# Nashatyrev/shadow

Measured on AMD Instinct MI355X. Metric: APSP wall time + source-SSSPs/sec, 10k-vertex GML graph, 1/2/4/8 MI355X, higher is better.
Workload: dtype u32+f32

## Files before the change

include/shadow_routing.h:

```cpp
#ifndef SHADOW_ROUTING_H
#define SHADOW_ROUTING_H

#include <stddef.h>
#include <stdint.h>

#ifdef __cplusplus
extern "C" {
#endif

#define SRG_OK 0
#define SRG_ERR_ARG 1
#define SRG_ERR_NO_EDGE 2
#define SRG_ERR_MULTI_EDGE 3
#define SRG_ERR_UNREACHABLE 4
#define SRG_ERR_LATENCY_RANGE 5
#define SRG_ERR_HIP 6
#define SRG_ERR_OOM 7
#define SRG_ERR_PARSE 8
#define SRG_ERR_RCCL 9
#define SRG_ERR_INTERNAL 10

typedef struct srg_edge_list {
    uint32_t num_vertices;
    uint32_t directed;
// ... 74 lines not shown
#define SRG_OPT_H2D_CODEC 25
#define SRG_OPT_EDGE_SHARD 29
#define SRG_OPT_LATE_LOSS 30
#define SRG_OPT_FW_LINE_SPLIT 31
#define SRG_OPT_FW_STEP 32
#define SRG_OPT_FW_OVERLAP 33
#define SRG_OPT_TEST_FAULT 34
#define SRG_OPT_TABLE_POOL_BYTES 35
#define SRG_OPT_TABLE_POOL_IDLE_BYTES 36
#define SRG_OPT_CREATE_MS_RUNTIME 37
#define SRG_OPT_CREATE_MS_LIBRARY 38
#define SRG_OPT_FW_XCD_ORDER 39
#define SRG_OPT_SCAN_MIRROR 40
#define SRG_OPT_SCAN_MIRRORED 41
#define SRG_OPT_SCAN_MIRROR_CAP 42
int srg_set_option(srg_ctx* ctx, int option, double value);
int srg_get_option(srg_ctx* ctx, int option, double* value);

int srg_compute_shortest_paths(srg_ctx* ctx, const srg_edge_list* graph,
                               const uint32_t* nodes, uint32_t num_nodes,
                               uint64_t* out_latency_ns, float* out_packet_loss,
                               srg_stats* stats, char* errbuf, size_t errlen);

int srg_compute_shortest_paths_device(srg_ctx* ctx, const srg_edge_list* graph_dev,
                                      const uint32_t* nodes_dev, uint32_t num_nodes,
                                      uint64_t* out_latency_ns_dev, float* out_packet_loss_dev,
                                      void* hip_stream, srg_stats* stats,
                                      char* errbuf, size_t errlen);

int srg_get_direct_paths(srg_ctx* ctx, const srg_edge_list* graph,
// ... 124 lines not shown
```

shadow_amd/_native.py:

```python
import ctypes
import os

_HERE = os.path.dirname(os.path.abspath(__file__))
LIB_PATH = os.path.join(_HERE, "libshadow_routing.so")

SRG_OK = 0
SRG_ERR_ARG = 1
SRG_ERR_NO_EDGE = 2
SRG_ERR_MULTI_EDGE = 3
SRG_ERR_UNREACHABLE = 4
SRG_ERR_LATENCY_RANGE = 5
SRG_ERR_HIP = 6
SRG_ERR_OOM = 7
SRG_ERR_PARSE = 8
SRG_ERR_RCCL = 9
SRG_ERR_INTERNAL = 10
SRG_ERR_EVENT_ORDER = 11

SRG_PATH_DENSE_U32 = 0
SRG_PATH_DENSE_U64 = 1
SRG_PATH_DIRECT = 2
SRG_PATH_SPARSE_U32 = 3
SRG_PATH_SPARSE_U64 = 4

# ... 13 lines not shown
SRG_OPT_H2D_CODEC = 25
SRG_OPT_EDGE_SHARD = 29
SRG_OPT_LATE_LOSS = 30
SRG_OPT_FW_LINE_SPLIT = 31
SRG_OPT_FW_STEP = 32
SRG_OPT_FW_OVERLAP = 33
SRG_OPT_TEST_FAULT = 34
SRG_OPT_TABLE_POOL_BYTES = 35
SRG_OPT_TABLE_POOL_IDLE_BYTES = 36
SRG_OPT_CREATE_MS_RUNTIME = 37
SRG_OPT_CREATE_MS_LIBRARY = 38
SRG_OPT_FW_XCD_ORDER = 39
SRG_OPT_SCAN_MIRROR = 40
SRG_OPT_SCAN_MIRRORED = 41
SRG_OPT_SCAN_MIRROR_CAP = 42
SRG_ALGO_AUTO = 0
SRG_ALGO_DENSE = 1
SRG_ALGO_SPARSE = 2
SRG_UNIQUE_ID_BYTES = 128

SRG_SCAN_NONE = 0
SRG_SCAN_SPARSE = 1
SRG_SCAN_DENSE = 2

_u32p = ctypes.POINTER(ctypes.c_uint32)
_u64p = ctypes.POINTER(ctypes.c_uint64)
_f32p = ctypes.POINTER(ctypes.c_float)


class EdgeList(ctypes.Structure):
# ... 249 lines not shown
```

shadow_amd/csrc/dense.hip.h:

```cpp
template <class K, int T>
bool run_dense(srg_ctx& c, const DevGraph& g, const Plan& pl, const uint32_t* nodes, uint32_t n, uint64_t* out_lat,
               float* out_loss, hipStream_t st, const Prelude& P, srg_stats* stats, HostSink* sink,
               FwOverlap* ov = nullptr) {
    const bool pre = ov && ov->on && ov->ok && ov->ended && sizeof(K) == 4 && T == FwOverlap::T;
    if (sizeof(K) == 8 && c.kout_key) {
        if (!(sink && sink->widen)) fail(SRG_INTERNAL_NEED_U64, "the build needs u64 latency keys: no u32 key table");
        sink->widen = false;
        c.kout_key = nullptr;
        c.kout_diag = nullptr;
    }
    const uint32_t V = g.V;
    const size_t Vp = ((size_t)V + T - 1) / T * T;
    const size_t VV = Vp * Vp;
    const bool multi = c.comm && c.comm->nranks > 1;
    Timer tm(st);
    c.own_row0 = pl.p0;
    c.own_row1 = pl.p1;

    K* W = (K*)c.b_W.get(VV * sizeof(K));
    uint32_t* WL = (uint32_t*)c.b_WL.get(VV * 4);
    K* D = (K*)c.b_D.get(VV * sizeof(K));
    bool wl_late = false;
    if (pre) {
        wl_late = g.late && !g.late->applied;
// ... 287 lines not shown
        const size_t Eb = E_layout + 256;
        uint32_t* cscpos = (uint32_t*)c.b_cscfill.get((size_t)nbTT5 * nK5 * V5_TT * 4);
        K* ent_w = (K*)c.b_entw.get(Eb * sizeof(K));
        uint2* ent_ub = (uint2*)c.b_grpe.get(Eb * 8);
        uint32_t* cscent = (uint32_t*)c.b_cscent.get(std::max<uint64_t>(E_ess, 1) * 4);
        k_v5_cscpos<<<(NT + 255) / 256, 256, 0, st>>>(v5_cnt, cscoff, NT, nK5, cscpos);
        uint2* rec = (uint2*)c.b_entkey.get((Eb + V5_SLACK) * 8);
        {
            const size_t nwaves = (size_t)nw64 * nK5;
            k_v5_fill<K><<<(unsigned)((nwaves * 64 + 255) / 256), 256, 0, st>>>(ess, W, WL, Vp, V, nw64, nK5, v5_cnt,
                                                                                  v5_goff, cscpos, rec, ent_w,
                                                                                  ent_ub, cscent);
        }
        HIP_CHECK(hipGetLastError());
        const size_t lds_rows = loss_rows_lds(V);
        bool mirror = c.scan_mirror && !g.directed && pl.G == 1 && !multi && !simulated && nloc == n && P.ident &&
                      !v5lo && lds_rows <= 150 * 1024;
        const uint32_t scan_groups = c.scan_groups ? (uint32_t)c.scan_groups : mirror ? 4u : 3u;
        const bool interleave = sink_rows && lds_rows <= 150 * 1024 && scan_groups > 1;
        if (interleave) set_lds(k_loss_rows<K, true>, lds_rows);
        uint32_t* PREDK = lds_rows <= 150 * 1024 ? (uint32_t*)c.b_PRED2.get(nmax * Vp * 8) : nullptr;
        auto pack_pred = [&](uint32_t r0, uint32_t r1) {
            const uint32_t nsb = (r1 - r0 + 127) / 128, nt8 = (nbTT5 + 7) / 8;
            k_pred_pack<<<8u * nt8 * nsb, 256, 0, st>>>(PRED, Vp, r0, r1, NT, nbTT5, nsb, ent_ub, (uint2*)PREDK,
                                                        multi_cnt, mirror ? 1u : 0u);
            HIP_CHECK(hipGetLastError());
        };
        auto mirror_rows = [&](uint32_t r0, uint32_t r1) {
            if (r1 <= r0 || r1 <= SB) return;
            const size_t pairs = (size_t)(r1 - r0) * Vp, room = std::min<size_t>(pairs / 2, (size_t)1 << 30);
            const uint32_t cap = (uint32_t)std::min<size_t>(
                room, c.scan_mirror_cap ? (size_t)c.scan_mirror_cap : std::max<size_t>(pairs / 1024, 256));
            uint2* work = (uint2*)(PRED + (size_t)r0 * Vp);
            HIP_CHECK(hipMemsetAsync(mirror_cnt, 0, 4, st));
            const uint32_t nlow = (r1 - 1) / SB * SB;
            k_pred_mirror<<<dim3(nlow / 64, (r1 - r0 + 63) / 64), 256, 0, st>>>((uint2*)PREDK, Vp, r0, r1, V, work, cap,
                                                                               mirror_cnt, multi_cnt);
            k_mirror_slow<K><<<1024, 256, 0, st>>>(work, mirror_cnt, cap, DST, npad, ent_ub, ent_w, cscoff, cscent,
                                                   (uint2*)PREDK, Vp, multi_cnt);
            HIP_CHECK(hipGetLastError());
        };
        std::vector<uint32_t> tri_h;
        if (nloc) HIP_CHECK(hipStreamWaitEvent(st, c.ev_dst, 0));
        for (bool again = nloc != 0; again;) {
            again = false;
            if (interleave) HIP_CHECK(hipMemsetAsync(&P.flags->changed, 0, 4, st));
            const uint32_t inf_check = v5lo ? 0u : 1u;
            const uint32_t nbS5 = (uint32_t)(npad / SB);
            const uint32_t ng = interleave ? std::min<uint32_t>(scan_groups, nbS5) : 1u;
            auto cut = [&](uint32_t q) { return mirror ? scan_group_cut_tri(q, ng, nbS5) : scan_group_cut(q, ng, nbS5); };
            const uint32_t* tri_d = nullptr;
            std::vector<size_t> tri_off(ng + 1, 0);
            if (mirror) {
                tri_h.clear();
                for (uint32_t gi = 0; gi < ng; ++gi) {
                    tri_scan_blocks(cut(gi), cut(gi + 1), nbTT5, tri_h);
                    tri_off[gi + 1] = tri_h.size();
                }
                uint32_t* d = (uint32_t*)c.b_tri.get(std::max<size_t>(tri_h.size(), 1) * 4);
                if (!tri_h.empty()) HIP_CHECK(hipMemcpyAsync(d, tri_h.data(), tri_h.size() * 4, hipMemcpyHostToDevice, st));
                HIP_CHECK(hipMemsetAsync(mirror_cnt, 0, 8, st));
                tri_d = d;
            }
            for (uint32_t gi = 0; gi < ng; ++gi) {
                const uint32_t c0 = cut(gi), c1 = cut(gi + 1);
                if (c1 == c0) continue;
                const uint32_t nblk = mirror ? (uint32_t)(tri_off[gi + 1] - tri_off[gi])
                                             : (nbTT5 + 3) / 4 * ((c1 - c0 + 7) / 8);
                if (nblk)
                    tight_v5<<<8u * 32u * ((nblk + 7) / 8), V5_WAVES * 64, 0, st>>>(
                        DSTs, npad, dsts_bytes, lnodes, nloc, V, NT, nbTT5, c1, nK5, c0, v5_goff,
                        (const uint32_t*)c.b_entkey.get(0), PRED, Vp, inf_check, mirror ? tri_d + tri_off[gi] : nullptr);
                HIP_CHECK(hipGetLastError());
                if (interleave) {
                    const uint32_t r0 = c0 * SB, r1 = std::min<uint32_t>(c1 * SB, nloc);
                    if (r1 <= r0) continue;
                    pack_pred(r0, r1);
                    if (mirror) mirror_rows(r0, r1);
                    k_loss_rows<K, true><<<r1 - r0, 1024, lds_rows, st>>>(PREDK, Vp, V, lnodes, nloc, ent_ub, ent_w,
                                                                   DST, npad, cscoff, cscent, P.selfloss, nodes, n,
                                                                   lpos, out_loss, &P.flags->changed, r0,
                                                                   mirror ? mirror_cnt + 1 : nullptr);
                    HIP_CHECK(hipGetLastError());
                    sink->send_rows(st, out_loss, sink->loss, pl.p0 + r0, r1 - r0, 4);
                }
            }
            if (!PREDK) k_count_multi<<<nloc, kThreads, 0, st>>>(PRED, nloc, V, Vp, multi_cnt);
            HIP_CHECK(hipGetLastError());
            ms_scan += tm.lap();
            if (interleave) {
                sink->loss_sent = true;
                rb_async(c, MS_CHANGED, &P.flags->changed, st);
                if (mirror) rb_async(c, MS_MIRROR, mirror_cnt + 1, st);
                HIP_CHECK(hipStreamSynchronize(st));
                rounds = (int)rb_get<uint32_t>(c, MS_CHANGED);
                loss_written = true;
            } else if (lds_rows <= 150 * 1024) {
                set_lds(k_loss_rows<K, true>, lds_rows);
                HIP_CHECK(hipMemsetAsync(&P.flags->changed, 0, 4, st));
                pack_pred(0, nloc);
                if (mirror) mirror_rows(0, nloc);
                const uint32_t nchunk = std::max<uint32_t>(1, std::min<uint32_t>(c.loss_chunks ? c.loss_chunks : sink_rows ? 8 : 1, nloc));
                for (uint32_t q = 0; q < nchunk; ++q) {
                    const uint32_t r0 = (uint32_t)((uint64_t)nloc * q / nchunk);
                    const uint32_t r1 = (uint32_t)((uint64_t)nloc * (q + 1) / nchunk);
                    if (r1 == r0) continue;
                    k_loss_rows<K, true><<<r1 - r0, 1024, lds_rows, st>>>(PREDK, Vp, V, lnodes, nloc, ent_ub, ent_w,
                                                                   DST, npad, cscoff, cscent, P.selfloss, nodes, n,
                                                                   lpos, out_loss, &P.flags->changed, r0,
                                                                   mirror ? mirror_cnt + 1 : nullptr);
                    HIP_CHECK(hipGetLastError());
                    if (sink_rows) sink->send_rows(st, out_loss, sink->loss, pl.p0 + r0, r1 - r0, 4);
                }
                if (sink_rows) sink->loss_sent = true;
                rb_async(c, MS_CHANGED, &P.flags->changed, st);
                if (mirror) rb_async(c, MS_MIRROR, mirror_cnt + 1, st);
                HIP_CHECK(hipStreamSynchronize(st));
                rounds = (int)rb_get<uint32_t>(c, MS_CHANGED);
                loss_written = true;
            } else {
                float* L0 = (float*)c.b_L0.get(nmax * Vp * 4);
                float* L1 = (float*)c.b_L1.get(nmax * Vp * 4);
// ... 103 lines not shown
```

shadow_amd/csrc/env_switches.h:

```cpp
#pragma once
#include <algorithm>
#include <cstddef>
#include <cstdlib>
#include <cstring>

namespace srg_env {

static inline bool is_set(const char* name) { return std::getenv(name) != nullptr; }
static inline bool first_char_is(const char* name, char ch) {
    const char* e = std::getenv(name);
    return e && e[0] == ch;
}
static inline bool equals(const char* name, const char* value) {
    const char* e = std::getenv(name);
    return e && std::strcmp(e, value) == 0;
}

static inline bool stream_hops_events() { return equals("SRG_STREAM_HOPS", "events"); }
static inline int fw_bulk_q() {
    const char* e = std::getenv("SRG_FW_BULK_Q");
    return !e ? -1 : e[0] == '0' ? 0 : e[0] == '1' ? 1 : -1;
}
static inline bool debug_overlap() { return is_set("SRG_DEBUG_OVERLAP"); }
static inline int debug_sparse() {
    const char* e = std::getenv("SRG_DEBUG_SPARSE");
    return !e ? 0 : e[0] == '2' ? 2 : 1;
}
static inline bool debug_codec() { return is_set("SRG_DEBUG_CODEC"); }
static inline bool debug_create() { return is_set("SRG_DEBUG_CREATE"); }
static inline bool sparse_kernel_bf() { return equals("SRG_SPARSE_KERNEL", "bf"); }
static inline bool sparse_split_off() { return first_char_is("SRG_SPARSE_SPLIT", '0'); }
static inline bool latency_unit_ns() { return equals("SRG_LATENCY_UNIT", "1"); }
static inline int codec_threads() {
// ... 15 lines not shown
```

shadow_amd/csrc/plan.h:

```cpp
#pragma once
#include <algorithm>
#include <cstddef>
#include <cstdint>
#include <vector>

namespace {

struct Plan {
    int G = 1, g = 0, nb = 0, rb0 = 0, rb1 = 0;
    std::vector<int> blk_lo;
    uint32_t p0 = 0, p1 = 0;
    std::vector<uint32_t> lnodes, lpos;
    int owner(int b) const { return (int)(std::upper_bound(blk_lo.begin(), blk_lo.end(), b) - blk_lo.begin()) - 1; }
    bool own(int b) const { return b >= rb0 && b < rb1; }
};

inline void tri_tile_h(int nb, int idx, int& I, int& J) {
    int i = 0;
    while (i + 1 < nb && (i + 1) * nb - (i + 1) * i / 2 <= idx) ++i;
    I = i;
    J = i + (idx - (i * nb - i * (i - 1) / 2));
}

inline Plan make_plan(int G, int g, uint32_t V, int T, const std::vector<uint32_t>& nodes_h) {
// ... 72 lines not shown
    if (q == 0) return 0u;
    if (q >= ng) return nblocks;
    const uint32_t last = nblocks ? (nblocks - 1) / 8 * 8 : 0u;
    const bool tail = ng >= 3 && last > 0;
    const uint32_t end = tail ? last : nblocks;
    const uint32_t parts = tail ? ng - 1 : ng;
    if (q >= parts) return end;
    const uint64_t want = tri_scan_work(end, nblocks) / 2;
    uint32_t c = 0;
    while (c < end && tri_scan_work(c, nblocks) < want) ++c;
    const uint32_t half = std::min(end, (c + 4) / 8 * 8);
    if (q == 1) return half;
    return std::min(end, half + ((end - half) * (q - 1) / (parts - 1) + 4) / 8 * 8);
}

}
```

shadow_amd/csrc/routing.hip:

```cpp
#include <hip/hip_runtime.h>
#include <hsa/hsa.h>
#include <hsa/hsa_ext_amd.h>
#include <sys/mman.h>

#include <algorithm>
#include <atomic>
#include <chrono>
#include <cmath>
#include <condition_variable>
#include <deque>
#include <cstdio>
#include <cstdlib>
#include <cstring>
#include <functional>
#include <map>
#include <memory>
#include <mutex>
#include <new>
#include <stdexcept>
#include <string>
#include <thread>
#include <vector>

#include "../../include/shadow_routing.h"
// ... 713 lines not shown
    Event ev_dst;
    int fw_line_split = 0;
    int fw_step = -1;
    DevBuf b_xlb, b_xflags;
    uint32_t xepoch = 0;
    std::vector<Event> ev_ov;
    uint32_t* kout_key = nullptr;
    uint64_t* kout_diag = nullptr;
    DevBuf b_odiag;
    int fw_overlap = 1;
    int fw_xcd_order = 1;
    int scan_mirror = 1;
    int scan_mirrored = 0;
    int scan_mirror_cap = 0;
    DevBuf b_tri;
    int test_fault = 0;
    std::shared_ptr<TablePool> tpool = std::make_shared<TablePool>();
    double ms_create_runtime = 0, ms_create_lib = 0;
    DevBuf b_ek0, b_ek1, b_eh0, b_eh1, b_ei0, b_ei1, b_ehist, b_eoffs, b_ered;
    ~srg_ctx() {
        delete comm;
        for (uint32_t* p : sig)
            if (p) (void)hipFree(p);
        if (h_lring) (void)hipHostFree(h_lring);
        if (hbox) (void)hipHostFree(hbox);
        for (hipStream_t s : {aux_stream, comm_stream, d2h_stream, stream})
            if (s) (void)hipStreamDestroy(s);
        delete pool;
        if (h_ring) (void)hipHostFree(h_ring);
        tpool->close();
// ... 77 lines not shown
                                      hipFuncAttributeMaxDynamicSharedMemorySize, (int)bytes));
}

constexpr int kMailSlots = 64;
template <class T>
void rb_async(srg_ctx& c, int slot, const T* dev, hipStream_t st) {
    static_assert(sizeof(T) <= 64, "mailbox slot");
    HIP_CHECK(hipMemcpyAsync(c.hbox + 64 * slot, dev, sizeof(T), hipMemcpyDeviceToHost, st));
}
template <class T>
T rb_get(const srg_ctx& c, int slot) {
    T v;
    std::memcpy(&v, c.hbox + 64 * slot, sizeof(T));
    return v;
}
enum MailSlot { MS_EDGESTATS, MS_FLAGS, MS_TIMEOUT, MS_REDUCE, MS_TAIL0, MS_TAIL1, MS_NMULTI, MS_CHANGED, MS_MIN, MS_REDUCE2, MS_MIRROR };

struct Prelude {
    EdgeStats es;
    uint32_t* selfcnt;
    uint64_t* selflat;
    float* selfloss;
    Flags* flags;
    std::vector<uint32_t> nodes_h;
    bool ident = false;
    bool range_risk = false;
    bool wrap_risk = false;
    uint64_t unit = 1;
    unsigned long long max_key = 0;
};

// ... 976 lines not shown
            fw->end(ms_xchg);
            ended = true;
        }
    }
};

#include "dense.hip.h"
#include "sparse_run.hip.h"

void compute_device(srg_ctx& c, const DevGraph& g, const uint32_t* nodes, uint32_t n, uint64_t* out_lat,
                    float* out_loss, hipStream_t st, srg_stats* stats, HostSink* sink = nullptr,
                    FwOverlap* ov = nullptr) {
    HIP_CHECK(hipStreamSynchronize(c.aux_stream));
    HIP_CHECK(hipStreamSynchronize(c.comm_stream));
    c.scan_mirrored = 0;
    if (g.V == 0) {
        if (n) fail(SRG_ERR_ARG, "nodes given for an empty graph");
        return;
    }
    const bool ov_fw = ov && ov->on && ov->ok && ov->begun;
    Prelude P = prelude(c, g, nodes, n, ov_fw ? c.comm_stream : st, true);
    if (n == 0) return;
    const uint64_t unit = (P.es.unit > 1 && !srg_env::latency_unit_ns()) ? P.es.unit : 1;
    P.unit = unit;
    const bool pre = ov && ov->on && ov->ok && ov->ended && P.es.max_lat < 0xFFFFFFFFull;
    if (pre) P.unit = 1;
    P.max_key = P.es.max_lat / P.unit;
    if (stats) stats->latency_unit_ns = P.unit;
    const unsigned __int128 bound = (unsigned __int128)P.max_key * (g.V > 1 ? g.V - 1 : 1);
    P.range_risk = bound >= ((unsigned __int128)1 << 62);
// ... 969 lines not shown
        lap("stream main");
        c->ms_create_runtime = ms_since(tcreate);
        const auto tlib = std::chrono::steady_clock::now();
        int prio_lo = 0, prio_hi = 0;
        HIP_CHECK(hipDeviceGetStreamPriorityRange(&prio_lo, &prio_hi));
        HIP_CHECK(hipStreamCreateWithPriority(&c->aux_stream, hipStreamNonBlocking, prio_hi));
        HIP_CHECK(hipStreamCreateWithFlags(&c->comm_stream, hipStreamNonBlocking));
        HIP_CHECK(hipStreamCreateWithFlags(&c->d2h_stream, hipStreamNonBlocking));
        lap("streams aux, comm, d2h");
        HIP_CHECK(hipHostMalloc((void**)&c->hbox, 64 * kMailSlots, hipHostMallocDefault));
        lap("mailbox");
        c->sdma.init(device);
        lap("sdma agents");
        c->loss_stream = c->d2h_stream;
        for (Event* e : {&c->ev_a, &c->ev_b, &c->ev_c, &c->ev_d, &c->ev_e, &c->ev_ledges, &c->ev_wlate, &c->ev_fwreset,
                         &c->ev_dst})
            e->create();
        int wv = 0;
        if (hipDeviceGetAttribute(&wv, hipDeviceAttributeCanUseStreamWaitValue, device) == hipSuccess && wv) {
            for (uint32_t*& p : c->sig) HIP_CHECK(hipExtMallocWithFlags((void**)&p, 8, hipMallocSignalMemory));
            HIP_CHECK(hipStreamWriteValue32(c->stream, c->sig[0], 0, 0));
            HIP_CHECK(hipStreamWriteValue32(c->stream, c->sig[1], 0, 0));
            HIP_CHECK(hipStreamSynchronize(c->stream));
        }
        lap("events, signals");
        if (!srg_env::create_warm_off()) {
            warm_context(*c);
            lap("warm-up (module, rings, copies)");
        }
        c->ms_create_lib = ms_since(tlib);
        std::lock_guard<std::mutex> lk(g_dev_mu);
// ... 93 lines not shown
#endif
            ctx->test_fault = (int)value;
            return SRG_OK;
        case SRG_OPT_FW_XCD_ORDER:
            if (value != 0 && value != 1) return SRG_ERR_ARG;
            ctx->fw_xcd_order = (int)value;
            return SRG_OK;
        case SRG_OPT_SCAN_MIRROR:
            if (value != 0 && value != 1) return SRG_ERR_ARG;
            ctx->scan_mirror = (int)value;
            return SRG_OK;
        case SRG_OPT_SCAN_MIRROR_CAP:
            if (!(value >= 0 && value <= 1073741824.0)) return SRG_ERR_ARG;
            ctx->scan_mirror_cap = (int)value;
            return SRG_OK;
        case SRG_OPT_TABLE_POOL_BYTES: {
            if (!(value >= 0.0 && value <= 1e15)) return SRG_ERR_ARG;
            std::lock_guard<std::mutex> pl(ctx->tpool->mu);
            ctx->tpool->limit = (size_t)value;
            ctx->tpool->max_idle = 0;
            ctx->tpool->trim_locked(ctx->tpool->limit);
            return SRG_OK;
        }
        case SRG_OPT_ALGORITHM:
            if (value != SRG_ALGO_AUTO && value != SRG_ALGO_DENSE && value != SRG_ALGO_SPARSE) return SRG_ERR_ARG;
            ctx->algorithm = (int)value;
            return SRG_OK;
        default:
            return SRG_ERR_ARG;
    }
// ... 26 lines not shown
            std::lock_guard<std::mutex> pl(ctx->tpool->mu);
            *value = (double)ctx->tpool->limit;
            break;
        }
        case SRG_OPT_TABLE_POOL_IDLE_BYTES: {
            std::lock_guard<std::mutex> pl(ctx->tpool->mu);
            *value = (double)ctx->tpool->idle_bytes;
            break;
        }
        case SRG_OPT_CREATE_MS_RUNTIME: *value = ctx->ms_create_runtime; break;
        case SRG_OPT_FW_XCD_ORDER: *value = ctx->fw_xcd_order; break;
        case SRG_OPT_CREATE_MS_LIBRARY: *value = ctx->ms_create_lib; break;
        case SRG_OPT_SCAN_MIRROR: *value = ctx->scan_mirror; break;
        case SRG_OPT_SCAN_MIRRORED: *value = ctx->scan_mirrored; break;
        case SRG_OPT_SCAN_MIRROR_CAP: *value = ctx->scan_mirror_cap; break;
        default: return SRG_ERR_ARG;
    }
    return SRG_OK;
}

void srg_destroy(srg_ctx* ctx) {
    if (!ctx) return;
    (void)hipSetDevice(ctx->device);
    {
        std::lock_guard<std::mutex> lk(g_dev_mu);
        --g_dev_ctx[ctx->device];
    }
    delete ctx;
}

// ... 424 lines not shown
```

shadow_amd/csrc/tight_sparse.hip.h:

```cpp
#pragma once
#include <hip/hip_runtime.h>
#include <stdint.h>

#include "kernels.hip.h"

namespace srg {

template <class K>
__global__ void __launch_bounds__(256) k_ess_mask(const K* __restrict__ W, const K* __restrict__ D, size_t ld,
                                                   uint32_t V, uint32_t u0, uint32_t u1, uint32_t nw64,
                                                   unsigned long long* __restrict__ ess) {
    const uint32_t lane = threadIdx.x & 63, wave = threadIdx.x >> 6;
    const uint32_t u = u0 + blockIdx.x;
    if (u >= u1) return;
    const K* Wu = W + (size_t)u * ld;
    const K* Du = D + (size_t)u * ld;
    unsigned long long* eu = ess + (size_t)u * nw64;
    if constexpr (sizeof(K) == 4) {
        for (uint32_t w0 = wave * 4; w0 < nw64; w0 += 16) {
            const uint32_t t = w0 * 64 + lane * 4;
            uint4 a = make_uint4(0u, 0u, 0u, 0u), d = make_uint4(1u, 1u, 1u, 1u);
            if (t < ld) {
                a = *reinterpret_cast<const uint4*>(Wu + t);
                d = *reinterpret_cast<const uint4*>(Du + t);
// ... 140 lines not shown
    if (j == V5_TW - 1) {
        const uint32_t total = incl;
        for (size_t q = 2 * ((size_t)pbase + total); q < 2 * (size_t)goff[g + 1]; ++q) {
            rec[q] = make_uint2(0u, KeyOps<uint32_t>::INF);
            ent_w[q] = KeyOps<K>::INF;
            ent_ub[q] = make_uint2(0u, __float_as_uint(1.0f));
        }
    }
}

typedef uint32_t v16u_v5 __attribute__((ext_vector_type(16)));
struct alignas(64) V5Grp {
    uint32_t v[16];
};

__global__ void __launch_bounds__(512, 4) tight_v5(const uint32_t* __restrict__ DST, size_t npad, uint32_t dst_bytes,
                                                    const uint32_t* __restrict__ nodes, uint32_t n, uint32_t V,
                                                    uint32_t NT, uint32_t nbTT, uint32_t nbS, uint32_t nK, uint32_t c0,
                                                    const uint32_t* __restrict__ goff, const uint32_t* __restrict__ rec,
                                                    uint32_t* __restrict__ PRED, size_t ldp, uint32_t inf_check,
                                                    const uint32_t* __restrict__ tri) {
    __shared__ __attribute__((aligned(16))) uint32_t rows[2 * V5_UC * V5_SB];
    const uint32_t bid = blockIdx.x, xcd = bid & 7, slot = bid >> 3;
    const uint32_t blk = (slot >> 5) * 8 + xcd, nbb = (nbTT + 3) / 4;
    uint32_t tb = blk % nbb, sg = blk / nbb;
    if (tri) {
        const uint32_t d = tri[blk];
        if (d == 0xFFFFFFFFu) return;
        tb = d & 0xFFFFu;
        sg = d >> 16;
    }
    const uint32_t b = tb * 4 + (slot & 3), c = c0 + sg * 8 + ((slot >> 2) & 7);
    if (c >= nbS || b >= nbTT) return;
    if (tri && b < c) return;
    const uint32_t tid = threadIdx.x, lane = tid & 63;
    const uint32_t wave = (uint32_t)__builtin_amdgcn_readfirstlane(tid >> 6);
    const uint32_t r0 = c * V5_SB + 2 * lane;
    const __amdgpu_buffer_rsrc_t rsrc = make_rsrc(DST, dst_bytes);
    const uint32_t t0 = b * V5_TT + wave * V5_TW;
// ... 88 lines not shown
    for (uint32_t h = 0; h < 2; ++h) {
        const uint32_t r = r0 + h;
        if (r >= n) continue;
        const uint32_t s = nodes[r];
        uint32_t o[V5_TW];
#pragma unroll
        for (uint32_t j = 0; j < V5_TW; ++j) {
            const uint32_t t = t0 + j;
            const uint32_t nd = h ? ndh[j] : ndl[j];
            const uint32_t st = h ? sth[j] : stl[j];
            o[j] = (t >= V || t == s || (inf_check && nd == 0u - KeyOps<uint32_t>::INF)) ? PRED_NONE : st;
        }
        uint4* out = reinterpret_cast<uint4*>(PRED + (size_t)r * ldp + t0);
#pragma unroll
        for (uint32_t j = 0; j < V5_TW; j += 4) out[j / 4] = make_uint4(o[j], o[j + 1], o[j + 2], o[j + 3]);
    }
}

__global__ void __launch_bounds__(256) k_pred_pack(const uint32_t* __restrict__ PRED, size_t ldp, uint32_t r0,
                                                   uint32_t r1, uint32_t NT, uint32_t nbTT, uint32_t nsb,
                                                   const uint2* __restrict__ ent_ub, uint2* __restrict__ PK,
                                                   unsigned long long* __restrict__ multi, uint32_t tri) {
    const uint32_t xcd = blockIdx.x & 7, slot = blockIdx.x >> 3;
    const uint32_t b = xcd + 8 * (slot / nsb), sb = slot % nsb;
    if (b >= nbTT) return;
    if (tri && b < r0 / V5_SB + sb) return;
    const uint32_t tx = threadIdx.x & 31, ty = threadIdx.x >> 5;
    const uint32_t t = b * V5_TT + tx * 4;
    const bool tv = t < NT;
    uint32_t nm = 0;
// ... 158 lines not shown
                const uint2 ub = ent_ub[e];
                if (KeyOps<K>::add(DST[(size_t)ub.x * npad + r], ent_w[e]) != dst) continue;
                const float cnd = fold_loss(Lrow[ub.x], __uint_as_float(ub.y));
                v = cnd < v ? cnd : v;
            }
        }
        Lout[r * ldp + t] = v;
        changed |= (v != Lrow[t]);
    }
    if (changed) atomicOr(changed_flag, 1u);
}

constexpr uint32_t U_SELF = 0xFFFFFFFFu, U_NONE = 0xFFFFFFFEu, U_MULTI = 0xFFFFFFFDu;
constexpr uint32_t U_MLIST = 0xF0000000u;
constexpr uint32_t LM_T = 32, LM_E = 16;
constexpr size_t loss_rows_lds(uint32_t V) { return (size_t)V * 12 + LM_T * (4 + 4 + LM_E * 8) + 16; }

template <class K, bool PK>
__global__ void __launch_bounds__(1024) k_loss_rows(const uint32_t* __restrict__ PRED, size_t ldp, uint32_t V,
                                                     const uint32_t* __restrict__ nodes, uint32_t n,
                                                     const uint2* __restrict__ ent_ub, const K* __restrict__ ent_w,
                                                     const K* __restrict__ DST, size_t npad,
                                                     const uint32_t* __restrict__ csc_off,
                                                     const uint32_t* __restrict__ csc_ent,
                                                     const float* __restrict__ self_loss,
                                                     const uint32_t* __restrict__ cols, uint32_t ncols,
                                                     const uint32_t* __restrict__ rowpos, float* __restrict__ out_loss,
                                                     uint32_t* __restrict__ max_sweeps, uint32_t row0,
                                                     const uint32_t* __restrict__ skip) {
    if (skip && *skip) return;
    extern __shared__ __attribute__((aligned(16))) unsigned char smem_raw[];
    uint32_t* U = reinterpret_cast<uint32_t*>(smem_raw);
    float* Bf = reinterpret_cast<float*>(U + V);
    float* L = Bf + V;
    uint32_t* m_t = reinterpret_cast<uint32_t*>(L + V);
    uint32_t* m_n = m_t + LM_T;
    uint32_t* m_u = m_n + LM_T;
    float* m_b = reinterpret_cast<float*>(m_u + LM_T * LM_E);
    __shared__ uint32_t changed, nm;
    const uint32_t r = row0 + blockIdx.x;
    const uint32_t s = nodes[r];
    const uint32_t* prow = PRED + (size_t)r * ldp * (PK ? 2 : 1);
    if (threadIdx.x == 0) nm = 0;
    if (threadIdx.x < LM_T) m_n[threadIdx.x] = 0;
    __syncthreads();
    for (uint32_t t = threadIdx.x; t < V; t += blockDim.x) {
        uint2 pk = make_uint2(0u, 0u);
        if constexpr (PK) pk = reinterpret_cast<const uint2*>(prow)[t];
        const uint32_t p = PK ? pk.x : prow[t];
        uint32_t u;
        float bb = 1.0f, l = 1.0f;
        if (t == s) {
            u = U_SELF;
            l = 0.0f;
        } else if (p == PRED_NONE) {
            u = U_NONE;
        } else if (p == PRED_MULTI) {
            const uint32_t i = atomicAdd(&nm, 1u);
            u = U_MULTI;
            if (i < LM_T) {
                m_t[i] = t;
                u = U_MLIST + i;
            }
        } else {
            const uint2 ub = PK ? pk : ent_ub[p];
            u = ub.x;
            bb = __uint_as_float(ub.y);
        }
        U[t] = u;
        Bf[t] = bb;
        L[t] = l;
    }
    __syncthreads();
    const uint32_t nml = nm < LM_T ? nm : LM_T;
    for (uint32_t i = 0; i < nml; ++i) {
        const uint32_t t = m_t[i];
        const K dst = DST[(size_t)t * npad + r];
        for (uint32_t k = csc_off[t] + threadIdx.x; k < csc_off[t + 1]; k += blockDim.x) {
            const uint32_t e = csc_ent[k];
            const uint2 ub = ent_ub[e];
            const uint32_t uu = ub.x;
            if (KeyOps<K>::add(DST[(size_t)uu * npad + r], ent_w[e]) != dst) continue;
            const uint32_t j = atomicAdd(&m_n[i], 1u);
            if (j < LM_E) {
                m_u[i * LM_E + j] = uu;
                m_b[i * LM_E + j] = __uint_as_float(ub.y);
            }
        }
    }
    __syncthreads();
    for (uint32_t i = threadIdx.x; i < nml; i += blockDim.x)
        if (m_n[i] > LM_E) U[m_t[i]] = U_MULTI;
    __syncthreads();
    uint32_t sweeps = 0;
    for (;;) {
        if (threadIdx.x == 0) changed = 0;
        __syncthreads();
        uint32_t ch = 0;
        for (uint32_t t = threadIdx.x; t < V; t += blockDim.x) {
            const uint32_t u = U[t];
            if (u >= U_MLIST) {
                if (u >= U_NONE) continue;
                float v = 1.0f;
                if (u == U_MULTI) {
                    const K dst = DST[(size_t)t * npad + r];
                    for (uint32_t k = csc_off[t]; k < csc_off[t + 1]; ++k) {
                        const uint32_t e = csc_ent[k];
                        const uint2 ub = ent_ub[e];
                        const uint32_t uu = ub.x;
                        if (KeyOps<K>::add(DST[(size_t)uu * npad + r], ent_w[e]) != dst) continue;
                        const float cnd = fold_loss(L[uu], __uint_as_float(ub.y));
                        v = cnd < v ? cnd : v;
                    }
                } else {
                    const uint32_t i = u - U_MLIST;
                    for (uint32_t j = 0; j < m_n[i]; ++j) {
                        const float cnd = fold_loss(L[m_u[i * LM_E + j]], m_b[i * LM_E + j]);
                        v = cnd < v ? cnd : v;
                    }
                }
                if (v != L[t]) {
                    L[t] = v;
                    ch = 1;
                }
                continue;
            }
            const float v = fold_loss(L[u], Bf[t]);
            if (v != L[t]) {
                L[t] = v;
                ch = 1;
            }
        }
        if (ch) changed = 1;
        __syncthreads();
        ++sweeps;
        if (!changed) break;
        __syncthreads();
    }
    if (threadIdx.x == 0) atomicMax(max_sweeps, sweeps);
    const uint32_t p = rowpos[r];
    float* orow = out_loss + (size_t)p * ncols;
    for (uint32_t j = threadIdx.x; j < ncols; j += blockDim.x) orow[j] = (j == p) ? self_loss[s] : L[cols[j]];
}

}
```

Before: 238,300.

## Stream tight scan into per-group loss passes; keep loss-row state in registers

Adds an opt-in streamed scan mode. A single tight_v5 launch on a side stream increments per-group completion counters, and the loss/pack/mirror work for each row group waits on those counters with a device-side spin kernel, so loss processing overlaps the rest of the scan instead of alternating with it. Separately, k_loss_rows now holds each thread's predecessor index and branch loss in register arrays (13 per thread), which shrinks its LDS footprint to just the L array. It also raises wave priority and adds a min-blocks launch bound, which should allow higher occupancy. The streaming path is off by default and depends on a spin-wait with a timeout, while the register rewrite always runs and increases register pressure.

```diff
diff --git a/include/shadow_routing.h b/include/shadow_routing.h
--- a/include/shadow_routing.h
+++ b/include/shadow_routing.h
@@ -112,6 +112,8 @@
 #define SRG_OPT_SCAN_MIRROR 40
 #define SRG_OPT_SCAN_MIRRORED 41
 #define SRG_OPT_SCAN_MIRROR_CAP 42
+#define SRG_OPT_SCAN_STREAM 43
+#define SRG_OPT_SCAN_STREAMED 44
 int srg_set_option(srg_ctx* ctx, int option, double value);
 int srg_get_option(srg_ctx* ctx, int option, double* value);
 
diff --git a/shadow_amd/_native.py b/shadow_amd/_native.py
--- a/shadow_amd/_native.py
+++ b/shadow_amd/_native.py
@@ -51,6 +51,8 @@
 SRG_OPT_SCAN_MIRROR = 40
 SRG_OPT_SCAN_MIRRORED = 41
 SRG_OPT_SCAN_MIRROR_CAP = 42
+SRG_OPT_SCAN_STREAM = 43
+SRG_OPT_SCAN_STREAMED = 44
 SRG_ALGO_AUTO = 0
 SRG_ALGO_DENSE = 1
 SRG_ALGO_SPARSE = 2
diff --git a/shadow_amd/csrc/dense.hip.h b/shadow_amd/csrc/dense.hip.h
--- a/shadow_amd/csrc/dense.hip.h
+++ b/shadow_amd/csrc/dense.hip.h
@@ -325,15 +325,23 @@
         }
         HIP_CHECK(hipGetLastError());
         const size_t lds_rows = loss_rows_lds(V);
+        const bool per_row = loss_rows_per_row(V);
         bool mirror = c.scan_mirror && !g.directed && pl.G == 1 && !multi && !simulated && nloc == n && P.ident &&
-                      !v5lo && lds_rows <= 150 * 1024;
+                      !v5lo && per_row;
+        bool stream_ok = c.scan_stream && sink_rows && per_row && pl.G == 1 && !multi && !simulated;
+        if (stream_ok) {
+            const bool events = srg_env::stream_hops_events();
+            std::lock_guard<std::mutex> lk(g_dev_mu);
+            stream_ok = g_dev_ctx[c.device] == 1 && !events;
+        }
         const uint32_t scan_groups = c.scan_groups ? (uint32_t)c.scan_groups : mirror ? 4u : 3u;
-        const bool interleave = sink_rows && lds_rows <= 150 * 1024 && scan_groups > 1;
+        const bool interleave = sink_rows && per_row && scan_groups > 1;
         if (interleave) set_lds(k_loss_rows<K, true>, lds_rows);
-        uint32_t* PREDK = lds_rows <= 150 * 1024 ? (uint32_t*)c.b_PRED2.get(nmax * Vp * 8) : nullptr;
+        uint32_t* PREDK = per_row ? (uint32_t*)c.b_PRED2.get(nmax * Vp * 8) : nullptr;
+        hipStream_t cst = st;
         auto pack_pred = [&](uint32_t r0, uint32_t r1) {
             const uint32_t nsb = (r1 - r0 + 127) / 128, nt8 = (nbTT5 + 7) / 8;
-            k_pred_pack<<<8u * nt8 * nsb, 256, 0, st>>>(PRED, Vp, r0, r1, NT, nbTT5, nsb, ent_ub, (uint2*)PREDK,
+            k_pred_pack<<<8u * nt8 * nsb, 256, 0, cst>>>(PRED, Vp, r0, r1, NT, nbTT5, nsb, ent_ub, (uint2*)PREDK,
                                                         multi_cnt, mirror ? 1u : 0u);
             HIP_CHECK(hipGetLastError());
         };
@@ -343,26 +351,81 @@
             const uint32_t cap = (uint32_t)std::min<size_t>(
                 room, c.scan_mirror_cap ? (size_t)c.scan_mirror_cap : std::max<size_t>(pairs / 1024, 256));
             uint2* work = (uint2*)(PRED + (size_t)r0 * Vp);
-            HIP_CHECK(hipMemsetAsync(mirror_cnt, 0, 4, st));
+            HIP_CHECK(hipMemsetAsync(mirror_cnt, 0, 4, cst));
             const uint32_t nlow = (r1 - 1) / SB * SB;
-            k_pred_mirror<<<dim3(nlow / 64, (r1 - r0 + 63) / 64), 256, 0, st>>>((uint2*)PREDK, Vp, r0, r1, V, work, cap,
+            k_pred_mirror<<<dim3(nlow / 64, (r1 - r0 + 63) / 64), 256, 0, cst>>>((uint2*)PREDK, Vp, r0, r1, V, work, cap,
                                                                                mirror_cnt, multi_cnt);
-            k_mirror_slow<K><<<1024, 256, 0, st>>>(work, mirror_cnt, cap, DST, npad, ent_ub, ent_w, cscoff, cscent,
+            k_mirror_slow<K><<<1024, 256, 0, cst>>>(work, mirror_cnt, cap, DST, npad, ent_ub, ent_w, cscoff, cscent,
                                                    (uint2*)PREDK, Vp, multi_cnt);
             HIP_CHECK(hipGetLastError());
         };
         std::vector<uint32_t> tri_h;
+        ScanStreamPlan sp;
+        std::vector<uint32_t> sp_h;
         if (nloc) HIP_CHECK(hipStreamWaitEvent(st, c.ev_dst, 0));
         for (bool again = nloc != 0; again;) {
             again = false;
             if (interleave) HIP_CHECK(hipMemsetAsync(&P.flags->changed, 0, 4, st));
             const uint32_t inf_check = v5lo ? 0u : 1u;
             const uint32_t nbS5 = (uint32_t)(npad / SB);
-            const uint32_t ng = interleave ? std::min<uint32_t>(scan_groups, nbS5) : 1u;
+            const bool try_stream = stream_ok && interleave && c.scan_mirrored != 2;
+            const uint32_t groups = try_stream && !c.scan_groups ? kScanStreamGroups : scan_groups;
+            const uint32_t ng = interleave ? std::min<uint32_t>(groups, nbS5) : 1u;
             auto cut = [&](uint32_t q) { return mirror ? scan_group_cut_tri(q, ng, nbS5) : scan_group_cut(q, ng, nbS5); };
             const uint32_t* tri_d = nullptr;
             std::vector<size_t> tri_off(ng + 1, 0);
-            if (mirror) {
+            bool streamed = false;
+            if (try_stream && ng > 1) {
+                std::vector<uint32_t> cuts(ng + 1);
+                for (uint32_t gi = 0; gi <= ng; ++gi) cuts[gi] = cut(gi);
+                streamed = scan_stream_plan(nbTT5, nbS5, cuts, mirror, sp) && sp.nblk > 0;
+            }
+            c.scan_streamed = streamed ? 1 : 0;
+            uint32_t *grp_done = nullptr, *scan_to = nullptr;
+            if (streamed) {
+                grp_done = (uint32_t*)c.b_scansync.get(((size_t)ng + 1) * 4);
+                scan_to = grp_done + ng;
+                HIP_CHECK(hipMemsetAsync(grp_done, 0, ((size_t)ng + 1) * 4, st));
+                sp_h = sp.tri;
+                sp_h.insert(sp_h.end(), sp.lo.begin(), sp.lo.end());
+                uint32_t* d = (uint32_t*)c.b_tri.get(sp_h.size() * 4);
+                HIP_CHECK(hipMemcpyAsync(d, sp_h.data(), sp_h.size() * 4, hipMemcpyHostToDevice, st));
+                if (mirror) HIP_CHECK(hipMemsetAsync(mirror_cnt, 0, 8, st));
+                const int on = srg_env::scan_stream_on();
+                hipStream_t ss = on == 2 ? c.aux_stream : c.comm_stream;
+                cst = on == 0 ? c.aux_stream : st;
+                HIP_CHECK(hipEventRecord(c.ev_scan0, st));
+                HIP_CHECK(hipStreamWaitEvent(ss, c.ev_scan0, 0));
+                if (cst != st) HIP_CHECK(hipStreamWaitEvent(cst, c.ev_scan0, 0));
+                tight_v5<<<8u * 32u * ((sp.nblk + 7) / 8), V5_WAVES * 64, 0, ss>>>(
+                    DSTs, npad, dsts_bytes, lnodes, nloc, V, NT, nbTT5, nbS5, nK5, 0u, v5_goff,
+                    (const uint32_t*)c.b_entkey.get(0), PRED, Vp, inf_check, mirror ? d : nullptr, grp_done,
+                    d + sp.tri.size(), ng);
+                HIP_CHECK(hipGetLastError());
+                HIP_CHECK(hipEventRecord(c.ev_scan1, ss));
+                const double ticks = 20.0 * (double)E_layout * (double)npad / 1e12 * 1e8;
+                const unsigned long long bound =
+                    std::max<unsigned long long>(200000000ull, (unsigned long long)std::min(ticks, 1e12));
+                for (uint32_t gi = 0; gi < ng; ++gi) {
+                    const uint32_t r0 = cut(gi) * SB, r1 = std::min<uint32_t>(cut(gi + 1) * SB, nloc);
+                    if (r1 <= r0) continue;
+                    k_hop_wait<<<1, 64, 0, cst>>>(grp_done + gi, sp.expect[gi] * V5_WAVES, scan_to, bound);
+                    pack_pred(r0, r1);
+                    if (mirror) mirror_rows(r0, r1);
+                    k_loss_rows<K, true><<<r1 - r0, LOSS_THREADS, lds_rows, cst>>>(
+                        PREDK, Vp, V, lnodes, nloc, ent_ub, ent_w, DST, npad, cscoff, cscent, P.selfloss, nodes, n, lpos,
+                        out_loss, &P.flags->changed, r0, mirror ? mirror_cnt + 1 : nullptr);
+                    HIP_CHECK(hipGetLastError());
+                    sink->send_rows(cst, out_loss, sink->loss, pl.p0 + r0, r1 - r0, 4);
+                }
+                HIP_CHECK(hipStreamWaitEvent(st, c.ev_scan1, 0));
+                if (cst != st) {
+                    HIP_CHECK(hipEventRecord(c.ev_scan2, cst));
+                    HIP_CHECK(hipStreamWaitEvent(st, c.ev_scan2, 0));
+                    cst = st;
+                }
+                rb_async(c, MS_SCANTO, scan_to, st);
+            } else if (mirror) {
                 tri_h.clear();
                 for (uint32_t gi = 0; gi < ng; ++gi) {
                     tri_scan_blocks(cut(gi), cut(gi + 1), nbTT5, tri_h);
@@ -373,7 +436,7 @@
                 HIP_CHECK(hipMemsetAsync(mirror_cnt, 0, 8, st));
                 tri_d = d;
             }
-            for (uint32_t gi = 0; gi < ng; ++gi) {
+            for (uint32_t gi = 0; gi < ng && !streamed; ++gi) {
                 const uint32_t c0 = cut(gi), c1 = cut(gi + 1);
                 if (c1 == c0) continue;
                 const uint32_t nblk = mirror ? (uint32_t)(tri_off[gi + 1] - tri_off[gi])
@@ -381,14 +444,15 @@
                 if (nblk)
                     tight_v5<<<8u * 32u * ((nblk + 7) / 8), V5_WAVES * 64, 0, st>>>(
                         DSTs, npad, dsts_bytes, lnodes, nloc, V, NT, nbTT5, c1, nK5, c0, v5_goff,
-                        (const uint32_t*)c.b_entkey.get(0), PRED, Vp, inf_check, mirror ? tri_d + tri_off[gi] : nullptr);
+                        (const uint32_t*)c.b_entkey.get(0), PRED, Vp, inf_check, mirror ? tri_d + tri_off[gi] : nullptr,
+                        nullptr, nullptr, 0u);
                 HIP_CHECK(hipGetLastError());
                 if (interleave) {
                     const uint32_t r0 = c0 * SB, r1 = std::min<uint32_t>(c1 * SB, nloc);
                     if (r1 <= r0) continue;
                     pack_pred(r0, r1);
                     if (mirror) mirror_rows(r0, r1);
-                    k_loss_rows<K, true><<<r1 - r0, 1024, lds_rows, st>>>(PREDK, Vp, V, lnodes, nloc, ent_ub, ent_w,
+                    k_loss_rows<K, true><<<r1 - r0, LOSS_THREADS, lds_rows, st>>>(PREDK, Vp, V, lnodes, nloc, ent_ub, ent_w,
                                                                    DST, npad, cscoff, cscent, P.selfloss, nodes, n,
                                                                    lpos, out_loss, &P.flags->changed, r0,
                                                                    mirror ? mirror_cnt + 1 : nullptr);
@@ -404,9 +468,11 @@
                 rb_async(c, MS_CHANGED, &P.flags->changed, st);
                 if (mirror) rb_async(c, MS_MIRROR, mirror_cnt + 1, st);
                 HIP_CHECK(hipStreamSynchronize(st));
+                if (streamed && rb_get<uint32_t>(c, MS_SCANTO))
+                    fail(SRG_ERR_HIP, "streamed scan: a group's wait for the scan launch timed out");
                 rounds = (int)rb_get<uint32_t>(c, MS_CHANGED);
                 loss_written = true;
-            } else if (lds_rows <= 150 * 1024) {
+            } else if (per_row) {
                 set_lds(k_loss_rows<K, true>, lds_rows);
                 HIP_CHECK(hipMemsetAsync(&P.flags->changed, 0, 4, st));
                 pack_pred(0, nloc);
@@ -416,7 +482,7 @@
                     const uint32_t r0 = (uint32_t)((uint64_t)nloc * q / nchunk);
                     const uint32_t r1 = (uint32_t)((uint64_t)nloc * (q + 1) / nchunk);
                     if (r1 == r0) continue;
-                    k_loss_rows<K, true><<<r1 - r0, 1024, lds_rows, st>>>(PREDK, Vp, V, lnodes, nloc, ent_ub, ent_w,
+                    k_loss_rows<K, true><<<r1 - r0, LOSS_THREADS, lds_rows, st>>>(PREDK, Vp, V, lnodes, nloc, ent_ub, ent_w,
                                                                    DST, npad, cscoff, cscent, P.selfloss, nodes, n,
                                                                    lpos, out_loss, &P.flags->changed, r0,
                                                                    mirror ? mirror_cnt + 1 : nullptr);
diff --git a/shadow_amd/csrc/env_switches.h b/shadow_amd/csrc/env_switches.h
--- a/shadow_amd/csrc/env_switches.h
+++ b/shadow_amd/csrc/env_switches.h
@@ -17,6 +17,9 @@
 }
 
 static inline bool stream_hops_events() { return equals("SRG_STREAM_HOPS", "events"); }
+static inline int scan_stream_on() {
+    return equals("SRG_SCAN_STREAM_ON", "comm") ? 1 : equals("SRG_SCAN_STREAM_ON", "aux") ? 2 : 0;
+}
 static inline int fw_bulk_q() {
     const char* e = std::getenv("SRG_FW_BULK_Q");
     return !e ? -1 : e[0] == '0' ? 0 : e[0] == '1' ? 1 : -1;
diff --git a/shadow_amd/csrc/plan.h b/shadow_amd/csrc/plan.h
--- a/shadow_amd/csrc/plan.h
+++ b/shadow_amd/csrc/plan.h
@@ -110,4 +110,47 @@
     return std::min(end, half + ((end - half) * (q - 1) / (parts - 1) + 4) / 8 * 8);
 }
 
+#if defined(__HIPCC__)
+#define SRG_PLAN_HD __host__ __device__
+#else
+#define SRG_PLAN_HD
+#endif
+SRG_PLAN_HD inline uint32_t scan_stream_group(uint32_t blk, const uint32_t* lo, uint32_t ng) {
+    uint32_t g = 0;
+    while (g + 1 < ng && lo[g + 1] <= blk) ++g;
+    return g;
 }
+constexpr uint32_t kScanStreamGroups = 4;
+struct ScanStreamPlan {
+    std::vector<uint32_t> tri;
+    std::vector<uint32_t> lo;
+    std::vector<uint32_t> expect;
+    uint32_t nblk = 0;
+};
+inline bool scan_stream_plan(uint32_t nbTT, uint32_t nbS, const std::vector<uint32_t>& cut, bool tri, ScanStreamPlan& p) {
+    const uint32_t ng = cut.empty() ? 0u : (uint32_t)cut.size() - 1, nbb = (nbTT + 3) / 4;
+    p.tri.clear();
+    p.lo.assign(ng + 1, 0);
+    p.expect.assign(ng, 0);
+    p.nblk = 0;
+    if (!ng || !nbTT || cut[0] != 0 || cut[ng] != nbS) return false;
+    for (uint32_t g = 0; g < ng; ++g)
+        if (cut[g + 1] < cut[g] || (g + 1 < ng && cut[g + 1] % 8 && cut[g + 1] != nbS)) return false;
+    for (uint32_t g = 0; g < ng; ++g) {
+        if (tri) {
+            const size_t base = p.tri.size();
+            tri_scan_blocks(cut[g], cut[g + 1], nbTT, p.tri);
+            for (size_t i = base; i < p.tri.size(); ++i)
+                if (p.tri[i] != TRI_PAD) p.tri[i] += cut[g] / 8 << 16;
+            p.lo[g + 1] = (uint32_t)p.tri.size();
+        } else {
+            p.lo[g + 1] = nbb * ((cut[g + 1] + 7) / 8);
+        }
+    }
+    p.nblk = p.lo[ng];
+    const uint32_t grid_blk = (p.nblk + 7) / 8 * 8;
+    for (uint32_t g = 0; g < ng; ++g) p.expect[g] = 32u * ((g + 1 < ng ? p.lo[g + 1] : grid_blk) - p.lo[g]);
+    return true;
+}
+
+}
diff --git a/shadow_amd/csrc/routing.hip b/shadow_amd/csrc/routing.hip
--- a/shadow_amd/csrc/routing.hip
+++ b/shadow_amd/csrc/routing.hip
@@ -751,6 +751,10 @@
     int scan_mirrored = 0;
     int scan_mirror_cap = 0;
     DevBuf b_tri;
+    int scan_stream = 0;
+    int scan_streamed = 0;
+    DevBuf b_scansync;
+    Event ev_scan0, ev_scan1, ev_scan2;
     int test_fault = 0;
     std::shared_ptr<TablePool> tpool = std::make_shared<TablePool>();
     double ms_create_runtime = 0, ms_create_lib = 0;
@@ -858,7 +862,7 @@
     std::memcpy(&v, c.hbox + 64 * slot, sizeof(T));
     return v;
 }
-enum MailSlot { MS_EDGESTATS, MS_FLAGS, MS_TIMEOUT, MS_REDUCE, MS_TAIL0, MS_TAIL1, MS_NMULTI, MS_CHANGED, MS_MIN, MS_REDUCE2, MS_MIRROR };
+enum MailSlot { MS_EDGESTATS, MS_FLAGS, MS_TIMEOUT, MS_REDUCE, MS_TAIL0, MS_TAIL1, MS_NMULTI, MS_CHANGED, MS_MIN, MS_REDUCE2, MS_MIRROR, MS_SCANTO };
 
 struct Prelude {
     EdgeStats es;
@@ -1865,6 +1869,7 @@
     HIP_CHECK(hipStreamSynchronize(c.aux_stream));
     HIP_CHECK(hipStreamSynchronize(c.comm_stream));
     c.scan_mirrored = 0;
+    c.scan_streamed = 0;
     if (g.V == 0) {
         if (n) fail(SRG_ERR_ARG, "nodes given for an empty graph");
         return;
@@ -2864,7 +2869,7 @@
         lap("sdma agents");
         c->loss_stream = c->d2h_stream;
         for (Event* e : {&c->ev_a, &c->ev_b, &c->ev_c, &c->ev_d, &c->ev_e, &c->ev_ledges, &c->ev_wlate, &c->ev_fwreset,
-                         &c->ev_dst})
+                         &c->ev_dst, &c->ev_scan0, &c->ev_scan1, &c->ev_scan2})
             e->create();
         int wv = 0;
         if (hipDeviceGetAttribute(&wv, hipDeviceAttributeCanUseStreamWaitValue, device) == hipSuccess && wv) {
@@ -2988,6 +2993,10 @@
             if (!(value >= 0 && value <= 1073741824.0)) return SRG_ERR_ARG;
             ctx->scan_mirror_cap = (int)value;
             return SRG_OK;
+        case SRG_OPT_SCAN_STREAM:
+            if (value != 0 && value != 1) return SRG_ERR_ARG;
+            ctx->scan_stream = (int)value;
+            return SRG_OK;
         case SRG_OPT_TABLE_POOL_BYTES: {
             if (!(value >= 0.0 && value <= 1e15)) return SRG_ERR_ARG;
             std::lock_guard<std::mutex> pl(ctx->tpool->mu);
@@ -3044,6 +3053,8 @@
         case SRG_OPT_SCAN_MIRROR: *value = ctx->scan_mirror; break;
         case SRG_OPT_SCAN_MIRRORED: *value = ctx->scan_mirrored; break;
         case SRG_OPT_SCAN_MIRROR_CAP: *value = ctx->scan_mirror_cap; break;
+        case SRG_OPT_SCAN_STREAM: *value = ctx->scan_stream; break;
+        case SRG_OPT_SCAN_STREAMED: *value = ctx->scan_streamed; break;
         default: return SRG_ERR_ARG;
     }
     return SRG_OK;
diff --git a/shadow_amd/csrc/tight_sparse.hip.h b/shadow_amd/csrc/tight_sparse.hip.h
--- a/shadow_amd/csrc/tight_sparse.hip.h
+++ b/shadow_amd/csrc/tight_sparse.hip.h
@@ -3,6 +3,7 @@
 #include <stdint.h>
 
 #include "kernels.hip.h"
+#include "plan.h"
 
 namespace srg {
 
@@ -178,15 +179,17 @@
     uint32_t v[16];
 };
 
-__global__ void __launch_bounds__(512, 4) tight_v5(const uint32_t* __restrict__ DST, size_t npad, uint32_t dst_bytes,
-                                                    const uint32_t* __restrict__ nodes, uint32_t n, uint32_t V,
-                                                    uint32_t NT, uint32_t nbTT, uint32_t nbS, uint32_t nK, uint32_t c0,
-                                                    const uint32_t* __restrict__ goff, const uint32_t* __restrict__ rec,
-                                                    uint32_t* __restrict__ PRED, size_t ldp, uint32_t inf_check,
-                                                    const uint32_t* __restrict__ tri) {
+__device__ __forceinline__ uint32_t v5_launch_block(uint32_t bid) { return ((bid >> 3) >> 5) * 8 + (bid & 7); }
+
+__device__ __forceinline__ void tight_v5_scan(const uint32_t* __restrict__ DST, size_t npad, uint32_t dst_bytes,
+                                              const uint32_t* __restrict__ nodes, uint32_t n, uint32_t V, uint32_t NT,
+                                              uint32_t nbTT, uint32_t nbS, uint32_t nK, uint32_t c0,
+                                              const uint32_t* __restrict__ goff, const uint32_t* __restrict__ rec,
+                                              uint32_t* __restrict__ PRED, size_t ldp, uint32_t inf_check,
+                                              const uint32_t* __restrict__ tri) {
     __shared__ __attribute__((aligned(16))) uint32_t rows[2 * V5_UC * V5_SB];
-    const uint32_t bid = blockIdx.x, xcd = bid & 7, slot = bid >> 3;
-    const uint32_t blk = (slot >> 5) * 8 + xcd, nbb = (nbTT + 3) / 4;
+    const uint32_t bid = blockIdx.x, slot = bid >> 3;
+    const uint32_t blk = v5_launch_block(bid), nbb = (nbTT + 3) / 4;
     uint32_t tb = blk % nbb, sg = blk / nbb;
     if (tri) {
         const uint32_t d = tri[blk];
@@ -305,6 +308,24 @@
         uint4* out = reinterpret_cast<uint4*>(PRED + (size_t)r * ldp + t0);
 #pragma unroll
         for (uint32_t j = 0; j < V5_TW; j += 4) out[j / 4] = make_uint4(o[j], o[j + 1], o[j + 2], o[j + 3]);
+    }
+}
+
+__global__ void __launch_bounds__(512, 4) tight_v5(const uint32_t* __restrict__ DST, size_t npad, uint32_t dst_bytes,
+                                                    const uint32_t* __restrict__ nodes, uint32_t n, uint32_t V,
+                                                    uint32_t NT, uint32_t nbTT, uint32_t nbS, uint32_t nK, uint32_t c0,
+                                                    const uint32_t* __restrict__ goff, const uint32_t* __restrict__ rec,
+                                                    uint32_t* __restrict__ PRED, size_t ldp, uint32_t inf_check,
+                                                    const uint32_t* __restrict__ tri, uint32_t* __restrict__ grp_done,
+                                                    const uint32_t* __restrict__ grp_lo, uint32_t ng) {
+    tight_v5_scan(DST, npad, dst_bytes, nodes, n, V, NT, nbTT, nbS, nK, c0, goff, rec, PRED, ldp, inf_check, tri);
+    if (!grp_done) return;
+    asm volatile("s_waitcnt vmcnt(0)" ::: "memory");
+    if (__builtin_amdgcn_mbcnt_hi(~0u, __builtin_amdgcn_mbcnt_lo(~0u, 0u)) == 0) {
+        __builtin_amdgcn_fence(__ATOMIC_RELEASE, "agent");
+        asm volatile("s_waitcnt vmcnt(0)" ::: "memory");
+        __hip_atomic_fetch_add(&grp_done[scan_stream_group(v5_launch_block(blockIdx.x), grp_lo, ng)], 1u,
+                               __ATOMIC_RELAXED, __HIP_MEMORY_SCOPE_AGENT);
     }
 }
 
@@ -493,10 +514,16 @@
 constexpr uint32_t U_SELF = 0xFFFFFFFFu, U_NONE = 0xFFFFFFFEu, U_MULTI = 0xFFFFFFFDu;
 constexpr uint32_t U_MLIST = 0xF0000000u;
 constexpr uint32_t LM_T = 32, LM_E = 16;
-constexpr size_t loss_rows_lds(uint32_t V) { return (size_t)V * 12 + LM_T * (4 + 4 + LM_E * 8) + 16; }
+constexpr uint32_t LOSS_THREADS = 1024;
+constexpr uint32_t LOSS_TPT = 13;
+constexpr size_t loss_rows_lists = LM_T * (4 + 4 + LM_E * 8) + 16;
+constexpr bool loss_rows_per_row(uint32_t V) { return (size_t)V * 12 + loss_rows_lists <= 150 * 1024; }
+constexpr size_t loss_rows_lds(uint32_t V) { return (size_t)V * 4 + loss_rows_lists; }
+static_assert(loss_rows_per_row(12436) && !loss_rows_per_row(12437) && 12436 <= LOSS_TPT * LOSS_THREADS,
+              "every eligible row's targets fit the register arrays");
 
 template <class K, bool PK>
-__global__ void __launch_bounds__(1024) k_loss_rows(const uint32_t* __restrict__ PRED, size_t ldp, uint32_t V,
+__global__ void __launch_bounds__(LOSS_THREADS, 8) k_loss_rows(const uint32_t* __restrict__ PRED, size_t ldp, uint32_t V,
                                                      const uint32_t* __restrict__ nodes, uint32_t n,
                                                      const uint2* __restrict__ ent_ub, const K* __restrict__ ent_w,
                                                      const K* __restrict__ DST, size_t npad,
@@ -508,10 +535,9 @@
                                                      uint32_t* __restrict__ max_sweeps, uint32_t row0,
                                                      const uint32_t* __restrict__ skip) {
     if (skip && *skip) return;
+    __builtin_amdgcn_s_setprio(3);
     extern __shared__ __attribute__((aligned(16))) unsigned char smem_raw[];
-    uint32_t* U = reinterpret_cast<uint32_t*>(smem_raw);
-    float* Bf = reinterpret_cast<float*>(U + V);
-    float* L = Bf + V;
+    float* L = reinterpret_cast<float*>(smem_raw);
     uint32_t* m_t = reinterpret_cast<uint32_t*>(L + V);
     uint32_t* m_n = m_t + LM_T;
     uint32_t* m_u = m_n + LM_T;
@@ -523,39 +549,47 @@
     if (threadIdx.x == 0) nm = 0;
     if (threadIdx.x < LM_T) m_n[threadIdx.x] = 0;
     __syncthreads();
-    for (uint32_t t = threadIdx.x; t < V; t += blockDim.x) {
-        uint2 pk = make_uint2(0u, 0u);
-        if constexpr (PK) pk = reinterpret_cast<const uint2*>(prow)[t];
-        const uint32_t p = PK ? pk.x : prow[t];
-        uint32_t u;
-        float bb = 1.0f, l = 1.0f;
-        if (t == s) {
-            u = U_SELF;
-            l = 0.0f;
-        } else if (p == PRED_NONE) {
-            u = U_NONE;
-        } else if (p == PRED_MULTI) {
-            const uint32_t i = atomicAdd(&nm, 1u);
-            u = U_MULTI;
-            if (i < LM_T) {
-                m_t[i] = t;
-                u = U_MLIST + i;
-            }
-        } else {
-            const uint2 ub = PK ? pk : ent_ub[p];
-            u = ub.x;
-            bb = __uint_as_float(ub.y);
-        }
-        U[t] = u;
-        Bf[t] = bb;
-        L[t] = l;
+    uint32_t Ur[LOSS_TPT];
+    float Br[LOSS_TPT];
+#pragma unroll
+    for (uint32_t i = 0; i < LOSS_TPT; ++i) {
+        const uint32_t t = threadIdx.x + LOSS_THREADS * i;
+        uint32_t u = U_NONE;
+        float bb = 1.0f;
+        if (t < V) {
+            uint2 pk = make_uint2(0u, 0u);
+            if constexpr (PK) pk = reinterpret_cast<const uint2*>(prow)[t];
+            const uint32_t p = PK ? pk.x : prow[t];
+            float l = 1.0f;
+            if (t == s) {
+                u = U_SELF;
+                l = 0.0f;
+            } else if (p == PRED_NONE) {
+                u = U_NONE;
+            } else if (p == PRED_MULTI) {
+                const uint32_t q = atomicAdd(&nm, 1u);
+                u = U_MULTI;
+                if (q < LM_T) {
+                    m_t[q] = t;
+                    u = U_MLIST + q;
+                }
+            } else {
+                const uint2 ub = PK ? pk : ent_ub[p];
+                u = ub.x * 4u;
+                bb = __uint_as_float(ub.y);
+            }
+            L[t] = l;
+        }
+        Ur[i] = u;
+        Br[i] = bb;
+        if ((i & 3) == 3) asm volatile("" ::: "memory");
     }
     __syncthreads();
     const uint32_t nml = nm < LM_T ? nm : LM_T;
     for (uint32_t i = 0; i < nml; ++i) {
         const uint32_t t = m_t[i];
         const K dst = DST[(size_t)t * npad + r];
-        for (uint32_t k = csc_off[t] + threadIdx.x; k < csc_off[t + 1]; k += blockDim.x) {
+        for (uint32_t k = csc_off[t] + threadIdx.x; k < csc_off[t + 1]; k += LOSS_THREADS) {
             const uint32_t e = csc_ent[k];
             const uint2 ub = ent_ub[e];
             const uint32_t uu = ub.x;
@@ -568,18 +602,23 @@
         }
     }
     __syncthreads();
-    for (uint32_t i = threadIdx.x; i < nml; i += blockDim.x)
-        if (m_n[i] > LM_E) U[m_t[i]] = U_MULTI;
-    __syncthreads();
+#pragma unroll
+    for (uint32_t i = 0; i < LOSS_TPT; ++i)
+        if (Ur[i] >= U_MLIST && Ur[i] < U_MULTI && m_n[Ur[i] - U_MLIST] > LM_E) Ur[i] = U_MULTI;
     uint32_t sweeps = 0;
     for (;;) {
         if (threadIdx.x == 0) changed = 0;
         __syncthreads();
         uint32_t ch = 0;
-        for (uint32_t t = threadIdx.x; t < V; t += blockDim.x) {
-            const uint32_t u = U[t];
+#pragma unroll
+        for (uint32_t i = 0; i < LOSS_TPT; ++i) {
+            if (threadIdx.x + LOSS_THREADS * i >= V) break;
+            uint32_t u = Ur[i];
+            asm volatile("" : "+v"(u));
             if (u >= U_MLIST) {
                 if (u >= U_NONE) continue;
+                uint32_t t = threadIdx.x + LOSS_THREADS * i;
+                asm volatile("" : "+v"(t));
                 float v = 1.0f;
                 if (u == U_MULTI) {
                     const K dst = DST[(size_t)t * npad + r];
@@ -592,9 +631,9 @@
                         v = cnd < v ? cnd : v;
                     }
                 } else {
-                    const uint32_t i = u - U_MLIST;
-                    for (uint32_t j = 0; j < m_n[i]; ++j) {
-                        const float cnd = fold_loss(L[m_u[i * LM_E + j]], m_b[i * LM_E + j]);
+                    const uint32_t q = u - U_MLIST;
+                    for (uint32_t j = 0; j < m_n[q]; ++j) {
+                        const float cnd = fold_loss(L[m_u[q * LM_E + j]], m_b[q * LM_E + j]);
                         v = cnd < v ? cnd : v;
                     }
                 }
@@ -604,7 +643,8 @@
                 }
                 continue;
             }
-            const float v = fold_loss(L[u], Bf[t]);
+            const uint32_t t = threadIdx.x + LOSS_THREADS * i;
+            const float v = fold_loss(*reinterpret_cast<const float*>(smem_raw + u), Br[i]);
             if (v != L[t]) {
                 L[t] = v;
                 ch = 1;
@@ -619,7 +659,7 @@
     if (threadIdx.x == 0) atomicMax(max_sweeps, sweeps);
     const uint32_t p = rowpos[r];
     float* orow = out_loss + (size_t)p * ncols;
-    for (uint32_t j = threadIdx.x; j < ncols; j += blockDim.x) orow[j] = (j == p) ? self_loss[s] : L[cols[j]];
-}
-
-}
+    for (uint32_t j = threadIdx.x; j < ncols; j += LOSS_THREADS) orow[j] = (j == p) ? self_loss[s] : L[cols[j]];
+}
+
+}
```

New measurement: 235,400. 1.2% lower.
